# lewisjiang/contour-context

Hardware: AMD Instinct MI355X
Metric: scans/sec ingest+query (120k-pt scan vs 5k-scan DB); max-F1 parity (higher is better)
Workload: dtype f32+f64

## Files before the change

### contour-context_amd/csrc/cont2_amd.hip

```cpp
#include <hip/hip_runtime.h>

#include <algorithm>
#include <array>
#include <chrono>
#include <cstdlib>
#include <climits>
#include <cmath>
#include <cstdio>
#include <cstring>
#include <string>
#include <condition_variable>
#include <mutex>
#include <thread>
#include <vector>

#include "../../include/cont2_amd.h"
#include "cc_hostcfg.h"
#include "k_rasterize.h"
#include "k_contours.h"
#include "k_contours_list.h"
#include "k_knn.h"
#include "k_check.h"
#include "k_merge.h"
#include "k_gmm.h"
// ... 358 lines not shown
    double ph[9] = {0}, sub[8] = {0}, lv[6] = {0}, sa[4] = {0};
    for (int i = 0; i < n; i++) {
      const long long *p = &h[(size_t)i * CC_K2_NCLK];
      ph[0] += p[1] * 0.01;
      ph[1] += p[2] * 0.01;
      ph[2] += p[3] * 0.01;
      ph[3] += (p[5] - p[4]) * 0.01;
      ph[4] += (p[6] - p[5]) * 0.01;
      ph[5] += (p[7] - p[6]) * 0.01;
      ph[6] += (p[8] - p[7]) * 0.01;
      ph[7] += (p[8] - p[0]) * 0.01;
      sub[0] += (p[9] - p[0]) * 0.01;
      sub[1] += (p[11] - p[10]) * 0.01;
      sub[2] += (p[12] - p[11]) * 0.01;
      sub[3] += (p[4] - p[12]) * 0.01;
      sub[4] += p[14] * 0.01;
      sub[5] += p[15] * 0.01;
      for (int j = 0; j < 6; j++) lv[j] += p[16 + j] * 0.01;
      sa[0] += (p[22] - p[0]) * 0.01;
      sa[1] += (p[23] - p[22]) * 0.01;
      sa[2] += (p[24] - p[23]) * 0.01;
      sa[3] += (p[9] - p[24]) * 0.01;
    }
    fprintf(stderr, "[cc_k_contours phases, mean us over %d scans] ccl %.1f  enum+bbox %.1f  walk %.1f  order+sort %.1f  emit %.1f  keys %.1f  bci %.1f  | total %.1f\n",
            n, ph[0] / n, ph[1] / n, ph[2] / n, ph[3] / n, ph[4] / n, ph[5] / n, ph[6] / n, ph[7] / n);
    fprintf(stderr, "[cc_k_contours sub-phases] fill+list %.1f | walk: member lists %.1f  lane walk %.1f  eight-lane walk %.1f | keys: RoI lists %.1f  division sums %.1f\n",
            sub[0] / n, sub[1] / n, sub[2] / n, sub[3] / n, sub[4] / n, sub[5] / n);
    {
      cc_k2_big_queue hq;
      HIPCHK(hipMemcpy(&hq, c->main.d_midq, sizeof(hq), hipMemcpyDeviceToHost));
      fprintf(stderr, "[cc_k_contours] scans handed to the mid path so far: %d (configuration %d, cells / slots %d, components %d, list padding %d)\n", hq.total, hq.why[0], hq.why[1], hq.why[2], hq.why[3]);
    }
    fprintf(stderr, "[cc_k_contours list stage A] levels %.1f  chunk ballots %.1f  prefix %.1f  entries + run labels %.1f\n", sa[0] / n, sa[1] / n, sa[2] / n, sa[3] / n);
    fprintf(stderr, "[cc_k_contours level loop, summed over the levels] unions %.1f  flatten+count %.1f  kept roots %.1f  rank %.1f  bbox/area %.1f  records %.1f\n",
            lv[0] / n, lv[1] / n, lv[2] / n, lv[3] / n, lv[4] / n, lv[5] / n);
  }
  ms_out[0] = c->ms_acc[0];
  ms_out[1] = c->ms_acc[1];
  if (n_launches) *n_launches = c->launches;
  c->ms_acc[0] = c->ms_acc[1] = 0;
  c->launches = 0;
  return CC_OK;
}

int cc_destroy(cc_ctx *c) {
#ifdef CC_TUNE_K1_CLK
  {
    unsigned long long h[8] = {0};
    if (hipMemcpyFromSymbol(h, HIP_SYMBOL(cc_k1_clk), sizeof h) == hipSuccess)
      fprintf(stderr, "[cc_k_rasterize clocks, ticks of 10 ns summed over workgroups (thread 0)] init %llu | A %llu | barrier %llu | B %llu | barrier %llu | emit %llu\n", h[0], h[1], h[2],
              h[3], h[4], h[5]);
  }
#endif
  if (!c) return CC_OK;
  hipSetDevice(c->device);
  for (auto &e : c->ev) hipEventDestroy(e);
  for (auto &ch : c->chan) {
    if (ch.s) {
      stream_give(c->device, ch.s);
    }
    hipFree(ch.d_pts);
    hipFree(ch.d_desc_tmp);
    hipFree(ch.d_bev_copy);
    scratch_free(ch.scr);
  }
  scratch_free(c->main);
  for (int i = 0; i < cc_ctx::NSLOT; i++) {
// ... 573 lines not shown
```

### contour-context_amd/csrc/k_contours.h

```cpp
#pragma once
#include "cc_dev.h"
#include "cc_group.h"
#include "cc_sort.h"
#include "cc_stats.h"
#include "cc_fmath.h"

#ifndef CC_OPAQUE_I
#define CC_OPAQUE_I(x) asm volatile("" : "+v"(x))
#endif

#define CC_NC CC_MAXC
#define CC_LAB_NONE 0xFFFFu
#define CC_LAB_PENDING 0x7FFEu

struct cc_comp_t {
  uint16_t root, area, parent, rank;
  uint8_t r0, r1, c0, c1, cA, cB, pad[2];
};

template <int NC>
struct cc_k2_scratch_t {
  cc_comp_t comp[CC_NLEV][NC];
  cc_contour_t cont[CC_NLEV][NC];
  alignas(16) uint16_t memb[CC_NLEV][((CC_MAX_CELLS + 7) & ~7) + 8 * NC];
// ... 143 lines not shown
    if (phase_clk) {                                                                      \
      const long long now_ = (long long)wall_clock64();                                   \
      if (tid == 0) phase_clk[(size_t)scan * CC_K2_NCLK + 16 + (j)] += now_ - tsub; \
      tsub = now_;                                                                        \
    }                                                                                     \
  } while (0)
#define CC_K2_LAP(acc)                                     \
  do {                                                     \
    if (phase_clk) {                                       \
      const long long now_ = (long long)wall_clock64();    \
      acc += now_ - tmark;                                 \
      tmark = now_;                                        \
    }                                                      \
  } while (0)

struct cc_k2_levmap {
  const unsigned char *LV;
  const unsigned long long *bitmap;
  const uint16_t *cbase;
  const unsigned char *lev;
  const uint16_t *g_rc;
  const float2 *g_pix;
  int n_act;
};
template <bool LISTED>
__device__ __forceinline__ int cc_k2_lev_at(const cc_k2_levmap &M, int cell) {
  if (!LISTED) return (int)M.LV[cell];
  const unsigned long long m = M.bitmap[cell >> 6];
  const int bit = cell & 63;
  if (!((m >> bit) & 1ull)) return 0;
  return (int)M.lev[(int)M.cbase[cell >> 6] + __popcll(m & ((1ull << bit) - 1ull))];
}

template <int NC, bool BIG, bool LISTED>
__device__ __forceinline__ void cc_k2_back(const cc_dev_cfg &cfg, const float2 *__restrict__ pix, const cc_k1_scan_out *__restrict__ k1_out,
                                           cc_k2_scratch_t<NC> *__restrict__ scr, cc_k2_big_tables *__restrict__ bigtab, int scan,
                                           cc_scan_desc_t *__restrict__ desc_out, int16_t *__restrict__ labels_dbg, long long *__restrict__ phase_clk,
                                           char *R, const int *n_lev_in, int flags_in, const cc_k2_levmap &lm) {
  const int n_cell = cfg.n_cell, n_col = cfg.n_col, n_row = cfg.n_row;
  const int tid = threadIdx.x, nt = blockDim.x;
  const int wave_id = tid >> 6, lane = tid & 63, n_waves = nt >> 6;
  cc_scan_desc_t *desc = desc_out + scan;
  long long tmark = 0;
  int n_lev[CC_NLEV];
  for (int l = 0; l < CC_NLEV; l++) n_lev[l] = n_lev_in[l];
#define CC_NLEV_AT(i) ((i) == 0 ? n_lev[0] : (i) == 1 ? n_lev[1] : (i) == 2 ? n_lev[2] : (i) == 3 ? n_lev[3] : (i) == 4 ? n_lev[4] : n_lev[5])
  const int flags0 = flags_in;
  cc_comp_t *T = BIG ? bigtab->T : (cc_comp_t *)R;
  unsigned *skey = BIG ? bigtab->skey : (unsigned *)(R + 30720);
  unsigned *arr = BIG ? bigtab->arr : (unsigned *)(R + 30720 + 7680);
  cc_anchor_lds *top = (cc_anchor_lds *)(R + 30720 + 2 * 7680);
  int *sh2 = (int *)(R + 30720 + 2 * 7680 + 1280);
  char *R2 = R + 30720 + 2 * 7680 + 1280 + 256;
  for (int l = 0; l < CC_NLEV; l++)
    for (int k = tid; k < n_lev[l]; k += nt) T[l * NC + k] = scr->comp[l][k];
  __syncthreads();
  for (int l = 0; l < CC_NLEV; l++) {
    const int n = n_lev[l];
    for (int k = tid; k < n; k += nt) {
      const cc_comp_t cp = T[l * NC + k];
      int py0 = 0, px0 = 0, prank = 0;
      if (l > 0) {
        unsigned p = cp.parent;
        if (p < (unsigned)n_lev[l - 1]) {
          const cc_comp_t pp = T[(l - 1) * NC + p];
          py0 = pp.r0;
          px0 = pp.c0;
          prank = pp.rank;
        }
      }
      const int rmin = cp.r0;
      const int brow = (rmin - py0) >> 1;
      const int ra = py0 + 2 * brow;
      int cm = cp.cA;
      if (ra == rmin && cp.cB < cm) cm = cp.cB;
      const int bcol = (cm - px0) >> 1;
      skey[l * NC + k] = ((unsigned)prank << 14) | ((unsigned)brow << 7) | (unsigned)bcol;
    }
    __syncthreads();
    for (int k0 = 0; k0 < n; k0 += nt >> 2) {
      const int k = k0 + (tid >> 2), q = tid & 3;
      const unsigned me = k < n ? skey[l * NC + k] : 0u;
      int rk = 0;
      for (int j = q; j < n; j += 4) rk += (skey[l * NC + j] < me) ? 1 : 0;
      rk += __shfl_xor(rk, 1);
      rk += __shfl_xor(rk, 2);
// ... 13 lines not shown
        [&]() {
          for (int k = lane; k < n; k += 64) a[T[l * NC + k].rank] = ((unsigned)T[l * NC + k].area << 16) | (unsigned)k;
        },
        lane, lpos, rasc, skey + l * NC, (unsigned *)R2 + l * CC_SORT_STACK);
    int tot = 0;
    for (int i = lane; i < n; i += 64) tot += (int)(a[i] >> 16);
    for (int o = 32; o > 0; o >>= 1) tot += __shfl_xor(tot, o);
    if (lane == 0) sh2[l] = tot;
  }
  __syncthreads();
  CC_K2_STAMP(5);
  for (int l = 0; l < CC_NLEV; l++) {
    const int n = n_lev[l] < CC_MAXC ? n_lev[l] : CC_MAXC;
    const int n_words = n * (int)(sizeof(cc_contour_t) / 4);
    const unsigned *src = (const unsigned *)&scr->cont[l][0];
    unsigned *dst = (unsigned *)&desc->cont[l][0];
    for (int w = tid; w < n_words; w += nt) {
      const int seq = w / 19, off = w - seq * 19;
      const int k = (int)(arr[l * NC + seq] & 0xFFFFu);
      dst[w] = src[k * 19 + off];
    }
    for (int seq = tid; seq < CC_NDIST && seq < n; seq += nt) {
      const int k = (int)(arr[l * NC + seq] & 0xFFFFu);
      const cc_contour_t *cv = &scr->cont[l][k];
      cc_anchor_lds a;
      a.pm[0] = cv->pos_mean[0];
      a.pm[1] = cv->pos_mean[1];
      a.ev[0] = cv->eig_vals[0];
      a.ev[1] = cv->eig_vals[1];
      a.cnt = cv->cell_cnt;
      top[l * CC_NDIST + seq] = a;
    }
  }
  if (tid < CC_NLEV) {
    desc->n_cont[tid] = CC_NLEV_AT(tid);
    desc->n_stored[tid] = CC_NLEV_AT(tid) < CC_MAXC ? CC_NLEV_AT(tid) : CC_MAXC;
    desc->layer_cell_cnt[tid] = sh2[tid];
  }
  if (tid == 0) {
    const cc_k1_scan_out k1 = k1_out[scan];
    desc->max_bin_val = k1.max_bin_val;
    desc->min_bin_val = k1.min_bin_val;
    desc->n_pix = k1.n_pix;
    int fl = flags0;
    for (int l = 0; l < CC_NLEV; l++) fl |= n_lev[l] > CC_MAXC ? CC_DESC_TRUNCATED : 0;
    desc->flags = fl;
  }
  if (labels_dbg) {
    for (int l = 0; l < CC_NLEV; l++)
      for (int seq = tid; seq < n_lev[l]; seq += nt) skey[l * NC + (arr[l * NC + seq] & 0xFFFFu)] = (unsigned)seq;
    __syncthreads();
    for (int l = 0; l < CC_NLEV; l++) {
      int16_t *ld = labels_dbg + ((size_t)scan * CC_NLEV + l) * n_cell;
      for (int c = tid; c < n_cell; c += nt) {
        int16_t v = ld[c];
        if (v >= 0) ld[c] = (int16_t)skey[l * NC + v];
      }
    }
  }
  __syncthreads();

  CC_K2_STAMP(6);
  float *divs = (float *)R2;
  int *cntp = (int *)(R2 + 5056);
  int *valid = cntp + 36;
  int *accum = valid + 36;
  const int NA = CC_NLEV * CC_NPIV;
  if (tid < NA) {
    const int ll = tid / CC_NPIV, seq = tid - ll * CC_NPIV;
    int ok = 0, acc = 0;
    if (seq < cfg.piv_firsts) {
      for (int s = 0; s <= seq; s++)
        if (s < CC_NLEV_AT(ll)) acc += top[ll * CC_NDIST + s].cnt;
      ok = (seq < CC_NLEV_AT(ll) && top[ll * CC_NDIST + seq].cnt >= cfg.min_cont_key_cnt) ? 1 : 0;
    }
    valid[tid] = ok;
    accum[tid] = acc;
    cntp[tid] = 0;
  }
  double *exp_tab = (double *)(R2 + 5504);
  unsigned char *vlist = (unsigned char *)(R2 + 5504 + 512);
  if (tid >= 64 && tid < 128) exp_tab[tid - 64] = __longlong_as_double((long long)cc_exp2_tab64[tid - 64]);
  __syncthreads();
  int NV = 0;
  for (int a = 0; a < CC_NLEV * CC_NPIV; a++) {
    const int ok = valid[a];
    if (ok && tid == 0) vlist[NV] = (unsigned char)a;
    NV += ok;
  }
  __syncthreads();
  const int roi_pad = (int)ceilf(cfg.roi_radius + 1.f);
  const float div_len = cfg.roi_radius / (float)(7 * 5);
  const float bin_len = cfg.roi_radius / (float)7;
  const double r_lim = (double)cfg.roi_radius - 1e-2;
// ... 239 lines not shown
      if (lane == 0) {
        bcnt[a] = n;
        ob->dist_bin[0] = bw[0];
        ob->dist_bin[1] = bw[1];
        ob->dist_bin[2] = bw[2];
        ob->dist_bin[3] = bw[3];
        ob->piv_seq = seq < cfg.piv_firsts ? (int8_t)seq : (int8_t)0;
        ob->level = seq < cfg.piv_firsts ? (int8_t)ll : (int8_t)0;
        ob->n_pts = (uint8_t)n;
        ob->n_segs = (uint8_t)ns;
      }
    }
  }
  __syncthreads();
  for (int t = tid; t < NA * CC_BCI_MAXPTS; t += nt) {
    const int a = t / CC_BCI_MAXPTS, i = t - a * CC_BCI_MAXPTS;
    const int ll = a / CC_NPIV, seq = a - ll * CC_NPIV;
    unsigned w0 = 0u;
    float r = 0.f, th = 0.f;
    if (i < bcnt[a]) {
      const unsigned k = bkey[a * CC_BCI_MAXPTS + i];
      const int q = (int)(k & 0xFFu);
      const bci_tmp o = btmp[a * CC_BCI_MAXPTS + q];
      w0 = (unsigned)(q / CC_NDIST + 1) | ((unsigned)(q % CC_NDIST) << 8) | ((k >> 8) << 16);
      r = o.r;
      th = o.theta;
    }
    unsigned *dst = (unsigned *)&desc->bcis[ll][seq].pts[i];
    dst[0] = w0;
    dst[1] = __float_as_uint(r);
    dst[2] = __float_as_uint(th);
  }
  CC_K2_STAMP(8);
}

template <int NC, bool BIG>
__device__ __forceinline__ void cc_k2_body(const cc_dev_cfg &cfg, const float *__restrict__ bev_in, const float2 *__restrict__ pix_in,
                                           const cc_k1_scan_out *__restrict__ k1_out, cc_k2_scratch_t<NC> *__restrict__ scr,
                                           cc_k2_big_tables *__restrict__ bigtab, cc_k2_big_queue *__restrict__ queue, int scan,
                                           cc_scan_desc_t *__restrict__ desc_out, int16_t *__restrict__ labels_dbg, long long *__restrict__ phase_clk,
                                           char *smem) {
  CC_K2_STAMP(0);
  const int n_cell = cfg.n_cell, n_col = cfg.n_col, n_row = cfg.n_row;
  const int tid = threadIdx.x, nt = blockDim.x;

  unsigned char *LV = (unsigned char *)smem;
  char *R = smem + CC_K2_LV_BYTES(n_cell);
  uint16_t *LAB = (uint16_t *)R;
  unsigned *W = BIG ? bigtab->W : (unsigned *)(R + 45056);
  uint16_t *roots = BIG ? bigtab->roots : (uint16_t *)(R + 45056 + 8960);
  uint16_t *cand = BIG ? bigtab->cand : roots + NC;
  uint16_t *prev_root = BIG ? bigtab->prev_root : cand + NC;
  int *sh = (int *)(R + 45056 + 8960 + 3 * CC_NC * 2 + 64);

  const float *bev = bev_in + (size_t)scan * n_cell;
  const float2 *pix = pix_in + (size_t)scan * n_cell;
  cc_scan_desc_t *desc = desc_out + scan;

  {
    const float4 *bev4 = (const float4 *)bev;
    const int n_quad = n_cell >> 2;
#pragma unroll 6
    for (int v = tid; v < n_quad; v += nt) {
      const float4 h4 = bev4[v];
      const float hh[4] = {h4.x, h4.y, h4.z, h4.w};
      unsigned lv4 = 0;
// ... 658 lines not shown
```

### contour-context_amd/csrc/k_contours_list.h

```cpp
#pragma once
#include "k_contours.h"

#define CC_K2L_NCAP CC_LIST_CAP
#define CC_K2L_SCAP 12800
#ifndef CC_K2L_MEMB
#define CC_K2L_MEMB 11264
#endif
#define CC_K2L_BIG 64
#define CC_K2L_WL_CAP (CC_K2L_MEMB / 2)
#define CC_K2L_NSTR (CC_K2L_NCAP / 64)
#define CC_K2L_NCHUNK ((CC_MAX_CELLS + 63) / 64)
#define CC_K2L_O_BITMAP 0
#define CC_K2L_O_CBASE 2816
#define CC_K2L_O_LEV 3584
#define CC_K2L_O_REST 6656
#define CC_K2L_R_RC 0
#define CC_K2L_R_X 6144
#define CC_K2L_R_MEMB 43008
#define CC_K2L_R_AREA (CC_K2L_R_MEMB + 2 * CC_K2L_MEMB)
#define CC_K2L_R_PTR (CC_K2L_R_AREA + 3840)
#define CC_K2L_R_SH (CC_K2L_R_PTR + 3840)
#define CC_K2L_LDS_BYTES (CC_K2L_O_REST + CC_K2L_R_SH + 1024)
#define CC_K2L_X_OFF (2 * CC_K2L_SCAP)
#define CC_K2L_X_BITA (CC_K2L_X_OFF + 2 * CC_K2L_NCAP + 16)
#define CC_K2L_X_BITB (CC_K2L_X_BITA + CC_K2L_SCAP / 8)
static_assert(CC_K2L_SCAP / CC_K2L_BIG <= 256 && CC_K2L_BIG == 64 && CC_K2L_SCAP % 32 == 0 && CC_K2L_X_BITA % 4 == 0 && CC_K2L_SCAP < 0x8000 && CC_K2L_NSTR <= 64 && CC_NC * CC_NLEV * 2 == 3840, "list front half: table sizes");
static_assert(CC_K2L_X_BITB + CC_K2L_SCAP / 8 <= 36864 && CC_K2L_NCAP * 12 <= 36864, "list front half: region X / stage A overlays");
static_assert(CC_K2L_R_SH >= CC_K2_R_BYTES, "the back half's region");

#ifdef CC_EMU
#define CC_K2L_TRACE_BAIL() do { if (getenv("CC_EMU_TRACE_K2")) fprintf(stderr, "[k2 list] scan %d handed to the mid path (line %d)\n", scan, __LINE__); } while (0)
#else
#define CC_K2L_TRACE_BAIL() do { } while (0)
#endif

__device__ __forceinline__ int cc_k2l_idx_of(const unsigned long long *bitmap, const uint16_t *cbase, int cell) {
  const unsigned long long m = bitmap[cell >> 6];
  const int bit = cell & 63;
  return ((m >> bit) & 1ull) ? (int)cbase[cell >> 6] + __popcll(m & ((1ull << bit) - 1ull)) : -1;
}

__device__ __forceinline__ unsigned cc_uf_find_h(uint16_t *LAB, unsigned x) {
  for (;;) {
    const unsigned p = cc_lds_vread16(LAB + x);
    if (p == x) return x;
    const unsigned gp = cc_lds_vread16(LAB + p);
    if (gp == p) return p;
    cc_lds_vwrite16(LAB + x, gp);
    x = gp;
  }
}
__device__ __forceinline__ void cc_uf_union_h(uint16_t *LAB, unsigned a, unsigned b) {
  a = cc_uf_find_h(LAB, a);
  b = cc_uf_find_h(LAB, b);
  while (a != b) {
    if (a < b) {
      const unsigned t = a;
      a = b;
      b = t;
    }
    unsigned *w = (unsigned *)LAB + (a >> 1);
// ... 41 lines not shown

  unsigned long long *bitmap = (unsigned long long *)(smem + CC_K2L_O_BITMAP);
  uint16_t *cbase = (uint16_t *)(smem + CC_K2L_O_CBASE);
  unsigned char *lev = (unsigned char *)(smem + CC_K2L_O_LEV);
  char *R = smem + CC_K2L_O_REST;
  uint16_t *rc = (uint16_t *)(R + CC_K2L_R_RC);
  char *X = R + CC_K2L_R_X;
  uint16_t *LAB = (uint16_t *)X;
  uint16_t *off = (uint16_t *)(X + CC_K2L_X_OFF);
  unsigned *bitA = (unsigned *)(X + CC_K2L_X_BITA), *bitB = (unsigned *)(X + CC_K2L_X_BITB);
  uint16_t *memb = (uint16_t *)(R + CC_K2L_R_MEMB);
  unsigned *wl = (unsigned *)(R + CC_K2L_R_MEMB);
  uint16_t *area = (uint16_t *)(R + CC_K2L_R_AREA);
  uint16_t *ptr = (uint16_t *)(R + CC_K2L_R_PTR);
  int *sh = (int *)(R + CC_K2L_R_SH);
  unsigned char *scnt = (unsigned char *)(R + CC_K2L_R_SH + 512);
  uint16_t *big = (uint16_t *)(R + CC_K2L_R_SH + 512);

  const float *bev = bev_in + (size_t)scan * n_cell;
  const float2 *pix = pix_in + (size_t)scan * n_cell;
  long long acc_ccl = 0, acc_enum = 0, acc_walk = 0, tmark = phase_clk ? (long long)wall_clock64() : 0, tsub = tmark;
  if (phase_clk && tid == 0)
    for (int j = 0; j < 6; j++) phase_clk[(size_t)scan * CC_K2_NCLK + 16 + j] = 0;

  const int4 hd = list.hdr[scan];
  const int n_act = hd.x, n_slot = hd.y;
#ifdef CC_EMU
  if (tid == 0 && getenv("CC_EMU_TRACE_K2")) fprintf(stderr, "[k2 list] scan %d: %d active cells, %d slots\n", scan, n_act, n_slot);
#endif
  if (n_act > CC_K2L_NCAP || n_slot > CC_K2L_SCAP) CC_K2L_BAIL(1);
  const int n_chunk = (n_cell + 63) >> 6;
  const int n_str = (n_act + 63) >> 6;
  uint16_t *ssum = (uint16_t *)scnt;
  {
    const uint16_t *g_rc = list.rc + (size_t)scan * CC_LIST_CAP;
    const unsigned char *g_lev = list.lev + (size_t)scan * CC_LIST_CAP;
    for (int i = tid; i < n_act; i += nt) {
      rc[i] = g_rc[i];
      lev[i] = g_lev[i];
    }
    for (int i = tid; i < n_chunk; i += nt) bitmap[i] = 0ull;
    if (tid < 128) sh[tid] = 0;
    if (labels_dbg)
      for (int i = tid; i < CC_NLEV * n_cell; i += nt) labels_dbg[(size_t)scan * CC_NLEV * n_cell + i] = (int16_t)-1;
  }
  __syncthreads();
  CC_K2_STAMP(22);
  for (int i = tid; i < n_act; i += nt) {
    const unsigned rcv = rc[i];
    const int c = (int)(rcv >> 8) * n_col + (int)(rcv & 255u);
    atomicOr(&bitmap[c >> 6], 1ull << (c & 63));
  }
  for (int q = wave_id; q < n_str; q += n_waves) {
    const int i = q * 64 + lane;
    int v = i < n_act ? (int)lev[i] : 0;
    for (int o = 32; o > 0; o >>= 1) v += __shfl_xor(v, o);
    if (lane == 0) ssum[q] = (uint16_t)v;
  }
  __syncthreads();
  CC_K2_STAMP(23);
  {
    const unsigned long long lane_le = lane_lt | (1ull << lane);
    int spre;
    {
      const int v = lane < n_str ? (int)ssum[lane] : 0;
      const int incl = cc_wave_scan_incl(v);
// ... 143 lines not shown
        LAB[oi + l] = (uint16_t)rt;
        const unsigned bit = 1u << (rt & 31u);
        if (atomicOr(&bitA[rt >> 5], bit) & bit) atomicOr(&bitB[rt >> 5], bit);
      }
    }
  }
  __syncthreads();
  CC_K2_SUBLAP(1);
  CC_K2_LAP(acc_ccl);
#define CC_K2L_KEPT(s_) (need <= 1 || (((need == 2 ? bitA : bitB)[(s_) >> 5] >> ((s_) & 31)) & 1u))
  for (int q = wave_id; q < n_str; q += n_waves) {
    const int i = q * 64 + lane;
    const int Li = i < n_act ? (int)lev[i] : 0, oi = i < n_act ? (int)off[i] : 0;
#pragma unroll
    for (int l = 0; l < CC_NLEV; l++) {
      const bool kp = l < Li && (unsigned)LAB[oi + l] == (unsigned)(oi + l) && CC_K2L_KEPT(oi + l);
      const unsigned long long m = __ballot(kp);
      if (lane == 0) scnt[l * CC_K2L_NSTR + q] = (unsigned char)__popcll(m);
    }
  }
  __syncthreads();
  CC_K2_SUBLAP(2);
  int nk[CC_NLEV], pre[CC_NLEV];
  bool too_many = false;
#pragma unroll
  for (int l = 0; l < CC_NLEV; l++) {
    const int v = lane < n_str ? (int)scnt[l * CC_K2L_NSTR + lane] : 0;
    const int incl = cc_wave_scan_incl(v);
    pre[l] = incl - v;
    nk[l] = cc_wave_scan_total(incl);
    too_many = too_many || nk[l] > NC;
  }
  if (too_many) CC_K2L_BAIL(2);
  for (int q = wave_id; q < n_str; q += n_waves) {
    const int i = q * 64 + lane;
    const int Li = i < n_act ? (int)lev[i] : 0, oi = i < n_act ? (int)off[i] : 0;
#pragma unroll
    for (int l = 0; l < CC_NLEV; l++) {
      const bool kp = l < Li && (unsigned)LAB[oi + l] == (unsigned)(oi + l) && CC_K2L_KEPT(oi + l);
      const unsigned long long m = __ballot(kp);
      const int base = __builtin_amdgcn_readlane(pre[l], q);
      if (kp) LAB[oi + l] = (uint16_t)(0x8000u | (unsigned)(base + cc_mbcnt(m)));
    }
  }
  __syncthreads();
  CC_K2_SUBLAP(3);
  for (int i = tid; i < n_act; i += nt) {
    const int Li = (int)lev[i], oi = (int)off[i];
    int16_t *ld = nullptr;
    int cell = 0;
    if (labels_dbg) {
      const unsigned rcv = rc[i];
      cell = (int)(rcv >> 8) * n_col + (int)(rcv & 255u);
      ld = labels_dbg + (size_t)scan * CC_NLEV * n_cell;
    }
    unsigned jprev = 0xFFFFu;
    for (int l = 0; l < Li; l++) {
      const unsigned v = LAB[oi + l];
      unsigned j = CC_COMP_NONE;
      if (v & 0x8000u) {
        j = v & 0x7FFFu;
        if (l > 0) scr->comp[l][j].parent = (uint16_t)jprev;
      } else if (v != (unsigned)(oi + l)) {
        const unsigned rv = LAB[v];
        if (rv & 0x8000u) {
          j = rv & 0x7FFFu;
          LAB[oi + l] = (uint16_t)rv;
        }
      }
      if (j != CC_COMP_NONE) {
        const unsigned t = (unsigned)(l * NC) + j;
        atomicAdd((unsigned *)area + (t >> 1), 1u << ((t & 1u) * 16));
        if (ld) ld[(size_t)l * n_cell + cell] = (int16_t)j;
      }
      jprev = j == CC_COMP_NONE ? 0xFFFFu : j;
    }
  }
  __syncthreads();
  CC_K2_SUBLAP(4);
  CC_K2_LAP(acc_enum);
#define CC_K2L_NK(l_) ((l_) == 0 ? nk[0] : (l_) == 1 ? nk[1] : (l_) == 2 ? nk[2] : (l_) == 3 ? nk[3] : (l_) == 4 ? nk[4] : nk[5])
  CC_K2_STAMP(10);
  for (int l = wave_id; l < CC_NLEV; l += n_waves) {
    const int n = CC_K2L_NK(l);
    int run = 0;
    for (int k0 = 0; k0 < n; k0 += 64) {
      const int k = k0 + lane;
      const int a = k < n ? (int)area[l * NC + k] : 0;
      const int a4 = (a + 1) & ~1;
      const int incl = cc_wave_scan_incl(a4);
      if (k < n) {
        ptr[l * NC + k] = (uint16_t)(run + incl - a4);
        const int cls = a >= CC_K2L_BIG ? 7 : 31 - __clz(a);
        atomicAdd(&sh[32 + cls], 1);
      }
      run += cc_wave_scan_total(incl);
    }
    if (lane == 0) sh[16 + l] = run;
  }
  __syncthreads();
  int lbase[CC_NLEV + 1];
  lbase[0] = 0;
#pragma unroll
  for (int l = 0; l < CC_NLEV; l++) lbase[l + 1] = lbase[l] + sh[16 + l];
  if (lbase[CC_NLEV] > CC_K2L_MEMB) CC_K2L_BAIL(3);
#define CC_K2L_LBASE(l_) ((l_) == 0 ? lbase[0] : (l_) == 1 ? lbase[1] : (l_) == 2 ? lbase[2] : (l_) == 3 ? lbase[3] : (l_) == 4 ? lbase[4] : lbase[5])
  float ch[CC_K2L_NCAP / CC_K2_BLOCK];
  float2 cp[CC_K2L_NCAP / CC_K2_BLOCK];
  static_assert(CC_K2L_NCAP % CC_K2_BLOCK == 0, "entries per thread");
#pragma unroll
  for (int u = 0; u < CC_K2L_NCAP / CC_K2_BLOCK; u++) {
    const int i = tid + u * CC_K2_BLOCK;
    ch[u] = 0.f;
    cp[u] = make_float2(0.f, 0.f);
// ... 45 lines not shown
        M &= bit ? B : ~B;
      }
      const int rank = cc_mbcnt(M), total = __popcll(M);
      const bool last = (M >> lane) == 1ull;
      int base = 0;
      if (j != CC_COMP_NONE) {
        base = (int)ptr_l[j];
        ml[base + rank] = (uint16_t)i;
      }
      cc_wave_sync();
      if (j != CC_COMP_NONE && last) ptr_l[j] = (uint16_t)(base + total);
      cc_wave_sync();
    }
  }
  __threadfence_block();
  __syncthreads();
  float *cbev = (float *)X;
  float2 *cpix = (float2 *)(X + CC_K2L_NCAP * 4);
#pragma unroll
  for (int u = 0; u < CC_K2L_NCAP / CC_K2_BLOCK; u++) {
    const int i = tid + u * CC_K2_BLOCK;
    if (i < n_act) {
      cbev[i] = ch[u];
      cpix[i] = cp[u];
    }
  }
  __syncthreads();
  CC_K2_STAMP(11);
  int lev_base[CC_NLEV + 1];
  lev_base[0] = 0;
#pragma unroll
  for (int l = 0; l < CC_NLEV; l++) lev_base[l + 1] = lev_base[l] + nk[l];
  const int n_tot = lev_base[CC_NLEV];
  auto finish_stats = [&](int l, int k, int a, const uint16_t *ml, const cc_running_stat &rec) {
    const unsigned rcl = rc[ml[a - 1]];
    cc_contour_t cvw;
    cc_calc_stat_vals(cfg, rec, l, (int)(rcl >> 8), (int)(rcl & 255u), &cvw);
    scr->cont[l][k] = cvw;
  };
  auto finish_shape = [&](int l, int k, int a, const uint16_t *ml, int c0, int c1, int cB) {
    const unsigned rc0 = rc[ml[0]];
    cc_comp_t *cpo = &scr->comp[l][k];
    const unsigned root_cell = (rc0 >> 8) * (unsigned)n_col + (rc0 & 255u);
    *(unsigned *)cpo = root_cell | ((unsigned)a << 16);
    cpo->rank = 0;
    cpo->r0 = (uint8_t)(rc0 >> 8);
    cpo->r1 = 0;
    cpo->c0 = (uint8_t)c0;
    cpo->c1 = (uint8_t)c1;
    cpo->cA = (uint8_t)(rc0 & 255u);
    cpo->cB = (uint8_t)cB;
    cpo->pad[0] = cpo->pad[1] = 0;
  };
  const int n_big = sh[40 + 7];
  const int half = nt >> 1;
  const bool lane_walker = tid < half || nt < 128;
  const int wt = nt < 128 ? tid : (tid < half ? tid : tid - half), wn = nt < 128 ? nt : half;
  if (lane_walker)
  for (int g = wt; g < n_big; g += wn) {
    const int t_ = (int)big[g];
    const int l = t_ / NC, k = t_ - l * NC;
    const int a = (int)area[t_];
    const uint16_t *ml = memb + CC_K2L_LBASE(l) + (int)ptr[t_] - a;
    const unsigned *mlw = (const unsigned *)ml;
    const int row1 = (int)(rc[ml[0]] >> 8) + 1;
    int c0 = 255, c1 = 0, cB = 255;
    for (int m0 = 0; m0 < a; m0 += 8) {
      const unsigned wds[4] = {mlw[m0 >> 1], mlw[(m0 >> 1) + 1], mlw[(m0 >> 1) + 2], mlw[(m0 >> 1) + 3]};
      const int nv = a - m0;
      unsigned rcu[8];
#pragma unroll
      for (int u = 0; u < 8; u++) rcu[u] = rc[((wds[u >> 1] >> ((u & 1) * 16)) & 0xFFFFu) & (unsigned)-(int)(u < nv)];
#pragma unroll
      for (int u = 0; u < 8; u++) {
        const int col = (int)(rcu[u] & 255u);
        if (u < nv) {
          c0 = col < c0 ? col : c0;
          c1 = col > c1 ? col : c1;
          cB = ((int)(rcu[u] >> 8) == row1 && col < cB) ? col : cB;
        }
      }
    }
    finish_shape(l, k, a, ml, c0, c1, cB);
  }
  const int n_small = n_tot - n_big;
  if (lane_walker)
  for (int w = wt; w < n_small; w += wn) {
    const int t_ = (int)scr->act[w];
    const int l = t_ / NC, k = t_ - l * NC;
    const int a = (int)area[t_];
    const uint16_t *ml = memb + CC_K2L_LBASE(l) + (int)ptr[t_] - a;
    const unsigned *mlw = (const unsigned *)ml;
    cc_running_stat rec;
    rec.cnt = a;
    rec.ps_x = rec.ps_y = rec.t_xx = rec.t_xy = rec.t_yy = rec.tq_x = rec.tq_y = 0.0;
    rec.vol3 = 0.f;
    const int row1 = (int)(rc[ml[0]] >> 8) + 1;
    int c0 = 255, c1 = 0, cB = 255;
    unsigned nx[4] = {mlw[0], mlw[1], mlw[2], mlw[3]};
    for (int m0 = 0; m0 < a; m0 += 8) {
      const unsigned wds[4] = {nx[0], nx[1], nx[2], nx[3]};
      if (m0 + 8 < a) {
#pragma unroll
        for (int u = 0; u < 4; u++) nx[u] = mlw[(m0 >> 1) + 4 + u];
      }
      const int nv = a - m0;
      unsigned mk[8], rcu[8];
      float hv[8];
      float2 rv[8];
#pragma unroll
      for (int u = 0; u < 8; u++) {
        mk[u] = (unsigned)-(int)(u < nv);
        const unsigned iu = ((wds[u >> 1] >> ((u & 1) * 16)) & 0xFFFFu) & mk[u];
        hv[u] = cbev[iu];
        rv[u] = cpix[iu];
        rcu[u] = rc[iu];
      }
#pragma unroll
      for (int u = 0; u < 8; u++) {
        const float h = __uint_as_float(__float_as_uint(hv[u]) & mk[u]);
        const double vr = (double)__uint_as_float(__float_as_uint(rv[u].x) & mk[u]);
        const double vc = (double)__uint_as_float(__float_as_uint(rv[u].y) & mk[u]);
        rec.ps_x += vr;
        rec.ps_y += vc;
        rec.t_xx += vr * vr;
        rec.t_xy += vr * vc;
        rec.t_yy += vc * vc;
        rec.vol3 += h;
        rec.tq_x += (double)h * vr;
        rec.tq_y += (double)h * vc;
        const int col = (int)(rcu[u] & 255u);
        const int colm = mk[u] ? col : 255;
        c0 = colm < c0 ? colm : c0;
        c1 = (mk[u] && col > c1) ? col : c1;
        cB = (mk[u] && (int)(rcu[u] >> 8) == row1 && cB == 255) ? col : cB;
      }
    }
    finish_stats(l, k, a, ml, rec);
    finish_shape(l, k, a, ml, c0, c1, cB);
  }
  CC_K2_STAMP(12);
  {
    const int role = tid & 7;
    const unsigned fa_h = role >= 5 ? ~0u : 0u, fa_y = (role == 1 || role == 4) ? ~0u : 0u, fa_x = ~(fa_h | fa_y);
    const unsigned fb_1 = role < 2 ? ~0u : 0u, fb_x = (role == 2 || role == 5) ? ~0u : 0u, fb_y = ~(fb_1 | fb_x);
    if (!lane_walker || nt < 128)
    for (int g0 = 0; g0 < n_big; g0 += wn >> 3) {
      const int g = g0 + (wt >> 3);
      const bool on = g < n_big;
      double acc = 0.0;
      float vol3 = 0.f;
      int l = 0, k = 0, a = 0;
      const uint16_t *ml = memb;
      if (on) {
        const int t = (int)big[g];
        l = t / NC;
        k = t - l * NC;
        a = (int)area[t];
        ml = memb + CC_K2L_LBASE(l) + (int)ptr[t] - a;
        const unsigned *mlw = (const unsigned *)ml;
        unsigned nx[4] = {mlw[0], mlw[1], mlw[2], mlw[3]};
        for (int m0 = 0; m0 < a; m0 += 8) {
          const unsigned wds[4] = {nx[0], nx[1], nx[2], nx[3]};
          if (m0 + 8 < a) {
#pragma unroll
            for (int u = 0; u < 4; u++) nx[u] = mlw[(m0 >> 1) + 4 + u];
          }
          const int nv = a - m0;
          unsigned mk[8];
          float hv[8];
          float2 rv[8];
#pragma unroll
// ... 25 lines not shown
      rec.vol3 = vol3;
      rec.cnt = a;
      if (on && role == 0) finish_stats(l, k, a, ml, rec);
    }
  }
  CC_K2_LAP(acc_walk);
  if (phase_clk && tid == 0) {
    phase_clk[(size_t)scan * CC_K2_NCLK + 1] = acc_ccl;
    phase_clk[(size_t)scan * CC_K2_NCLK + 2] = acc_enum;
    phase_clk[(size_t)scan * CC_K2_NCLK + 3] = acc_walk;
  }
  CC_K2_STAMP(4);
#pragma unroll
  for (int l = 0; l < CC_NLEV; l++) n_lev_out[l] = nk[l];
  return true;
#undef CC_K2L_BAIL
#undef CC_K2L_KEPT
#undef CC_K2L_NK
#undef CC_K2L_LBASE
}

__global__ void __launch_bounds__(CC_K2_BLOCK, 4)
cc_k_contours(cc_dev_cfg cfg, const float *__restrict__ bev_in, const float2 *__restrict__ pix_in,
              const cc_k1_scan_out *__restrict__ k1_out, cc_k2_scratch *__restrict__ scratch_all,
              cc_scan_desc_t *__restrict__ desc_out, int16_t *__restrict__ labels_dbg, long long *__restrict__ phase_clk,
              cc_k2_big_queue *__restrict__ midq, cc_k1_list_out list) {
  HIP_DYNAMIC_SHARED(char, smem)
  const int scan = (int)blockIdx.x;
  cc_k2_scratch *scr = scratch_all + scan;
  int n_lev[CC_NLEV];
  if (!cc_k2_front_list(cfg, bev_in, pix_in, scr, midq, scan, desc_out, labels_dbg, phase_clk, smem, n_lev, list)) return;
  __threadfence_block();
  __syncthreads();
  cc_k2_levmap lm;
  lm.LV = nullptr;
  lm.bitmap = (const unsigned long long *)(smem + CC_K2L_O_BITMAP);
  lm.cbase = (const uint16_t *)(smem + CC_K2L_O_CBASE);
  lm.lev = (const unsigned char *)(smem + CC_K2L_O_LEV);
  lm.g_rc = list.rc + (size_t)scan * CC_LIST_CAP;
  lm.g_pix = list.pix + (size_t)scan * CC_LIST_CAP;
  lm.n_act = list.hdr[scan].x;
  cc_k2_back<CC_NC, false, true>(cfg, pix_in + (size_t)scan * cfg.n_cell, k1_out, scr, nullptr, scan, desc_out, labels_dbg, phase_clk,
                                 smem + CC_K2L_O_REST, n_lev, 0, lm);
}

__global__ void __launch_bounds__(CC_K2_BLOCK, 2)
cc_k_contours_mid(cc_dev_cfg cfg, float *bev_io, float2 *pix_io ,
                  const cc_k1_scan_out *__restrict__ k1_out, cc_k2_scratch *__restrict__ scratch_all, cc_k2_big_queue *__restrict__ midq,
                  cc_k2_big_queue *__restrict__ bigq, cc_scan_desc_t *__restrict__ desc_out, int16_t *__restrict__ labels_dbg,
                  int *__restrict__ seen ,
                  cc_k1_list_out list) {
  HIP_DYNAMIC_SHARED(char, smem)
  __shared__ int s_next;
  if (midq->n_flagged == 0) {
    if (blockIdx.x == 0 && threadIdx.x == 0) *seen = 0;
    return;
  }
  for (;;) {
    __syncthreads();
    if (threadIdx.x == 0) s_next = atomicAdd(&midq->next, 1);
    __syncthreads();
    const int k = s_next;
    if (k >= midq->n_flagged) {
      if (threadIdx.x == 0 && atomicAdd(&midq->exited, 1) == (int)gridDim.x - 1) {
        *seen = midq->n_flagged;
        midq->n_flagged = 0;
        midq->next = 0;
        midq->exited = 0;
      }
      return;
    }
    const int scan = midq->scan[k];
    const int4 hd = list.hdr[scan];
    if (hd.z == 0) {
#ifdef CC_EMU
      if (threadIdx.x == 0 && getenv("CC_EMU_TRACE_K2")) fprintf(stderr, "[k2 mid] scan %d: dense image rebuilt from the list (%d entries)\n", scan, hd.x);
// ... 49 lines not shown
```

Baseline: 598,800.

## Order and sort contours inside the list kernel, write records directly to descriptor

The list contour kernel now computes each kept component's geometry (top row, min column, row-below min column) with atomics during the label pass. It then ranks components by parent-relative position and sorts them by area in shared memory. Contour statistics are written straight into the output descriptor at their final sequence index, so the separate back-half pass (copy to scratch, rank, sort, gather) is skipped. This also removes the per-component member walks for shape bounds and the extra global scratch traffic. In exchange it adds LDS atomics and an O(n^2/4) rank loop, and it relies on new shared-memory overlays that must not collide.

```diff
diff --git a/contour-context_amd/csrc/cont2_amd.hip b/contour-context_amd/csrc/cont2_amd.hip
--- a/contour-context_amd/csrc/cont2_amd.hip
+++ b/contour-context_amd/csrc/cont2_amd.hip
@@ -414,7 +414,7 @@
       fprintf(stderr, "[cc_k_contours] scans handed to the mid path so far: %d (configuration %d, cells / slots %d, components %d, list padding %d)\n", hq.total, hq.why[0], hq.why[1], hq.why[2], hq.why[3]);
     }
     fprintf(stderr, "[cc_k_contours list stage A] levels %.1f  chunk ballots %.1f  prefix %.1f  entries + run labels %.1f\n", sa[0] / n, sa[1] / n, sa[2] / n, sa[3] / n);
-    fprintf(stderr, "[cc_k_contours level loop, summed over the levels] unions %.1f  flatten+count %.1f  kept roots %.1f  rank %.1f  bbox/area %.1f  records %.1f\n",
+    fprintf(stderr, "[cc_k_contours level loop, summed over the levels] unions %.1f  flatten+count %.1f  kept roots %.1f  rank %.1f  bbox/area %.1f  records (list kernel: order + sort) %.1f\n",
             lv[0] / n, lv[1] / n, lv[2] / n, lv[3] / n, lv[4] / n, lv[5] / n);
   }
   ms_out[0] = c->ms_acc[0];
diff --git a/contour-context_amd/csrc/k_contours.h b/contour-context_amd/csrc/k_contours.h
--- a/contour-context_amd/csrc/k_contours.h
+++ b/contour-context_amd/csrc/k_contours.h
@@ -199,6 +199,33 @@
   return (int)M.lev[(int)M.cbase[cell >> 6] + __popcll(m & ((1ull << bit) - 1ull))];
 }
 
+#define CC_K2_R_TOP (30720 + 2 * 7680)
+
+__device__ __forceinline__ void cc_k2_header(const cc_k1_scan_out *__restrict__ k1_out, int scan, cc_scan_desc_t *__restrict__ desc,
+                                             const int *n_lev, const int *lcc, int flags0) {
+  const int tid = threadIdx.x;
+#define CC_NLEV_AT(i) ((i) == 0 ? n_lev[0] : (i) == 1 ? n_lev[1] : (i) == 2 ? n_lev[2] : (i) == 3 ? n_lev[3] : (i) == 4 ? n_lev[4] : n_lev[5])
+  if (tid < CC_NLEV) {
+    desc->n_cont[tid] = CC_NLEV_AT(tid);
+    desc->n_stored[tid] = CC_NLEV_AT(tid) < CC_MAXC ? CC_NLEV_AT(tid) : CC_MAXC;
+    desc->layer_cell_cnt[tid] = lcc[tid];
+  }
+#undef CC_NLEV_AT
+  if (tid == 0) {
+    const cc_k1_scan_out k1 = k1_out[scan];
+    desc->max_bin_val = k1.max_bin_val;
+    desc->min_bin_val = k1.min_bin_val;
+    desc->n_pix = k1.n_pix;
+    int fl = flags0;
+    for (int l = 0; l < CC_NLEV; l++) fl |= n_lev[l] > CC_MAXC ? CC_DESC_TRUNCATED : 0;
+    desc->flags = fl;
+  }
+}
+
+template <bool LISTED>
+__device__ __forceinline__ void cc_k2_keys_bci(const cc_dev_cfg &cfg, const float2 *__restrict__ pix, int scan, cc_scan_desc_t *__restrict__ desc,
+                                               long long *__restrict__ phase_clk, char *R, const int *n_lev_in, const cc_k2_levmap &lm);
+
 template <int NC, bool BIG, bool LISTED>
 __device__ __forceinline__ void cc_k2_back(const cc_dev_cfg &cfg, const float2 *__restrict__ pix, const cc_k1_scan_out *__restrict__ k1_out,
                                            cc_k2_scratch_t<NC> *__restrict__ scr, cc_k2_big_tables *__restrict__ bigtab, int scan,
@@ -216,9 +243,9 @@
   cc_comp_t *T = BIG ? bigtab->T : (cc_comp_t *)R;
   unsigned *skey = BIG ? bigtab->skey : (unsigned *)(R + 30720);
   unsigned *arr = BIG ? bigtab->arr : (unsigned *)(R + 30720 + 7680);
-  cc_anchor_lds *top = (cc_anchor_lds *)(R + 30720 + 2 * 7680);
-  int *sh2 = (int *)(R + 30720 + 2 * 7680 + 1280);
-  char *R2 = R + 30720 + 2 * 7680 + 1280 + 256;
+  cc_anchor_lds *top = (cc_anchor_lds *)(R + CC_K2_R_TOP);
+  int *sh2 = (int *)(R + CC_K2_R_TOP + 1280);
+  char *R2 = R + CC_K2_R_TOP + 1280 + 256;
   for (int l = 0; l < CC_NLEV; l++)
     for (int k = tid; k < n_lev[l]; k += nt) T[l * NC + k] = scr->comp[l][k];
   __syncthreads();
@@ -298,20 +325,7 @@
       top[l * CC_NDIST + seq] = a;
     }
   }
-  if (tid < CC_NLEV) {
-    desc->n_cont[tid] = CC_NLEV_AT(tid);
-    desc->n_stored[tid] = CC_NLEV_AT(tid) < CC_MAXC ? CC_NLEV_AT(tid) : CC_MAXC;
-    desc->layer_cell_cnt[tid] = sh2[tid];
-  }
-  if (tid == 0) {
-    const cc_k1_scan_out k1 = k1_out[scan];
-    desc->max_bin_val = k1.max_bin_val;
-    desc->min_bin_val = k1.min_bin_val;
-    desc->n_pix = k1.n_pix;
-    int fl = flags0;
-    for (int l = 0; l < CC_NLEV; l++) fl |= n_lev[l] > CC_MAXC ? CC_DESC_TRUNCATED : 0;
-    desc->flags = fl;
-  }
+  cc_k2_header(k1_out, scan, desc, n_lev, sh2, flags0);
   if (labels_dbg) {
     for (int l = 0; l < CC_NLEV; l++)
       for (int seq = tid; seq < n_lev[l]; seq += nt) skey[l * NC + (arr[l * NC + seq] & 0xFFFFu)] = (unsigned)seq;
@@ -325,7 +339,23 @@
     }
   }
   __syncthreads();
-
+  cc_k2_keys_bci<LISTED>(cfg, pix, scan, desc, phase_clk, R, n_lev, lm);
+#undef CC_NLEV_AT
+}
+
+template <bool LISTED>
+__device__ __forceinline__ void cc_k2_keys_bci(const cc_dev_cfg &cfg, const float2 *__restrict__ pix, int scan, cc_scan_desc_t *__restrict__ desc,
+                                               long long *__restrict__ phase_clk, char *R, const int *n_lev_in, const cc_k2_levmap &lm) {
+  const int n_cell = cfg.n_cell, n_col = cfg.n_col, n_row = cfg.n_row;
+  const int tid = threadIdx.x, nt = blockDim.x;
+  const int wave_id = tid >> 6, lane = tid & 63, n_waves = nt >> 6;
+  long long tmark = 0;
+  int n_lev[CC_NLEV];
+  for (int l = 0; l < CC_NLEV; l++) n_lev[l] = n_lev_in[l];
+#define CC_NLEV_AT(i) ((i) == 0 ? n_lev[0] : (i) == 1 ? n_lev[1] : (i) == 2 ? n_lev[2] : (i) == 3 ? n_lev[3] : (i) == 4 ? n_lev[4] : n_lev[5])
+  const cc_anchor_lds *top = (const cc_anchor_lds *)(R + CC_K2_R_TOP);
+  char *R2 = R + CC_K2_R_TOP + 1280 + 256;
+  (void)n_cell;
   CC_K2_STAMP(6);
   float *divs = (float *)R2;
   int *cntp = (int *)(R2 + 5056);
@@ -631,6 +661,7 @@
     dst[2] = __float_as_uint(th);
   }
   CC_K2_STAMP(8);
+#undef CC_NLEV_AT
 }
 
 template <int NC, bool BIG>
diff --git a/contour-context_amd/csrc/k_contours_list.h b/contour-context_amd/csrc/k_contours_list.h
--- a/contour-context_amd/csrc/k_contours_list.h
+++ b/contour-context_amd/csrc/k_contours_list.h
@@ -24,9 +24,17 @@
 #define CC_K2L_X_OFF (2 * CC_K2L_SCAP)
 #define CC_K2L_X_BITA (CC_K2L_X_OFF + 2 * CC_K2L_NCAP + 16)
 #define CC_K2L_X_BITB (CC_K2L_X_BITA + CC_K2L_SCAP / 8)
+#define CC_K2L_X_GEO (CC_K2L_X_BITA + 4 * CC_NLEV * CC_NC)
+#define CC_K2L_X_C0 (CC_K2L_X_GEO + 2 * CC_NLEV * CC_NC)
+#define CC_K2L_X_CB (CC_K2L_X_C0 + 4 * CC_NLEV * CC_NC)
+#define CC_K2L_X_STK (CC_K2L_X_CB + 4 * CC_NLEV * CC_NC)
 static_assert(CC_K2L_SCAP / CC_K2L_BIG <= 256 && CC_K2L_BIG == 64 && CC_K2L_SCAP % 32 == 0 && CC_K2L_X_BITA % 4 == 0 && CC_K2L_SCAP < 0x8000 && CC_K2L_NSTR <= 64 && CC_NC * CC_NLEV * 2 == 3840, "list front half: table sizes");
 static_assert(CC_K2L_X_BITB + CC_K2L_SCAP / 8 <= 36864 && CC_K2L_NCAP * 12 <= 36864, "list front half: region X / stage A overlays");
 static_assert(CC_K2L_R_SH >= CC_K2_R_BYTES, "the back half's region");
+static_assert(CC_K2L_X_GEO >= CC_K2L_X_BITB + CC_K2L_SCAP / 8 && CC_K2L_X_GEO >= CC_K2L_R_MEMB - CC_K2L_R_X && CC_K2L_X_C0 % 4 == 0 &&
+              CC_K2L_X_STK + 4 * CC_NLEV * CC_SORT_STACK <= CC_K2L_R_AREA - CC_K2L_R_X && CC_NC <= 512 && 2 * CC_NC * 2 <= 4 * CC_NC,
+              "list front half: the ordering tables (GEO / C0 / CB are written in (D), while bitA / bitB are still read; they end "
+              "before the areas; a sort's two u16 lists fit a CB row)");
 
 #ifdef CC_EMU
 #define CC_K2L_TRACE_BAIL() do { if (getenv("CC_EMU_TRACE_K2")) fprintf(stderr, "[k2 list] scan %d handed to the mid path (line %d)\n", scan, __LINE__); } while (0)
@@ -134,6 +142,12 @@
   const int n_chunk = (n_cell + 63) >> 6;
   const int n_str = (n_act + 63) >> 6;
   uint16_t *ssum = (uint16_t *)scnt;
+  unsigned *ARR = (unsigned *)(X + CC_K2L_X_BITA);
+  uint16_t *GEO = (uint16_t *)(X + CC_K2L_X_GEO);
+  unsigned *C0 = (unsigned *)(X + CC_K2L_X_C0);
+  unsigned *CB = (unsigned *)(X + CC_K2L_X_CB);
+  unsigned *STK = (unsigned *)(X + CC_K2L_X_STK);
+  uint16_t *PAR = ptr;
   {
     const uint16_t *g_rc = list.rc + (size_t)scan * CC_LIST_CAP;
     const unsigned char *g_lev = list.lev + (size_t)scan * CC_LIST_CAP;
@@ -343,6 +357,7 @@
     too_many = too_many || nk[l] > NC;
   }
   if (too_many) CC_K2L_BAIL(2);
+#define CC_K2L_NK(l_) ((l_) == 0 ? nk[0] : (l_) == 1 ? nk[1] : (l_) == 2 ? nk[2] : (l_) == 3 ? nk[3] : (l_) == 4 ? nk[4] : nk[5])
   for (int q = wave_id; q < n_str; q += n_waves) {
     const int i = q * 64 + lane;
     const int Li = i < n_act ? (int)lev[i] : 0, oi = i < n_act ? (int)off[i] : 0;
@@ -351,27 +366,29 @@
       const bool kp = l < Li && (unsigned)LAB[oi + l] == (unsigned)(oi + l) && CC_K2L_KEPT(oi + l);
       const unsigned long long m = __ballot(kp);
       const int base = __builtin_amdgcn_readlane(pre[l], q);
-      if (kp) LAB[oi + l] = (uint16_t)(0x8000u | (unsigned)(base + cc_mbcnt(m)));
+      if (kp) {
+        const int j = base + cc_mbcnt(m);
+        LAB[oi + l] = (uint16_t)(0x8000u | (unsigned)j);
+        GEO[l * NC + j] = rc[i];
+        C0[l * NC + j] = 255u;
+        CB[l * NC + j] = 255u;
+      }
     }
   }
   __syncthreads();
   CC_K2_SUBLAP(3);
   for (int i = tid; i < n_act; i += nt) {
     const int Li = (int)lev[i], oi = (int)off[i];
-    int16_t *ld = nullptr;
-    int cell = 0;
-    if (labels_dbg) {
-      const unsigned rcv = rc[i];
-      cell = (int)(rcv >> 8) * n_col + (int)(rcv & 255u);
-      ld = labels_dbg + (size_t)scan * CC_NLEV * n_cell;
-    }
+    const unsigned rcv = rc[i];
+    const int col = (int)(rcv & 255u), row = (int)(rcv >> 8);
+    const int lw = (col > 0 && i > 0 && (unsigned)rc[i - 1] == rcv - 1u) ? (int)lev[i - 1] : 0;
     unsigned jprev = 0xFFFFu;
     for (int l = 0; l < Li; l++) {
       const unsigned v = LAB[oi + l];
       unsigned j = CC_COMP_NONE;
       if (v & 0x8000u) {
         j = v & 0x7FFFu;
-        if (l > 0) scr->comp[l][j].parent = (uint16_t)jprev;
+        if (l > 0) PAR[l * NC + j] = (uint16_t)jprev;
       } else if (v != (unsigned)(oi + l)) {
         const unsigned rv = LAB[v];
         if (rv & 0x8000u) {
@@ -382,15 +399,100 @@
       if (j != CC_COMP_NONE) {
         const unsigned t = (unsigned)(l * NC) + j;
         atomicAdd((unsigned *)area + (t >> 1), 1u << ((t & 1u) * 16));
-        if (ld) ld[(size_t)l * n_cell + cell] = (int16_t)j;
+        if (l >= lw) {
+          atomicMin(&C0[t], (unsigned)col);
+          if (row == (int)(GEO[t] >> 8) + 1) atomicMin(&CB[t], (unsigned)col);
+        }
       }
       jprev = j == CC_COMP_NONE ? 0xFFFFu : j;
     }
   }
   __syncthreads();
   CC_K2_SUBLAP(4);
+  for (int l = 0; l < CC_NLEV; l++) {
+    const int n = CC_K2L_NK(l);
+    const int np = l > 0 ? CC_K2L_NK(l - 1) : 0;
+    for (int k = tid; k < n; k += nt) {
+      const int t = l * NC + k;
+      int py0 = 0, px0 = 0, prank = 0;
+      if (l > 0) {
+        const unsigned p = PAR[t];
+        if (p < (unsigned)np) {
+          const unsigned pc = C0[(l - 1) * NC + p];
+          py0 = (int)(GEO[(l - 1) * NC + p] >> 8);
+          px0 = (int)(pc & 255u);
+          prank = (int)(pc >> 16);
+        }
+      }
+      const unsigned g = GEO[t];
+      const int rmin = (int)(g >> 8);
+      const int brow = (rmin - py0) >> 1;
+      const int ra = py0 + 2 * brow;
+      int cm = (int)(g & 255u);
+      const int cb = (int)CB[t];
+      if (ra == rmin && cb < cm) cm = cb;
+      const int bcol = (cm - px0) >> 1;
+      CB[t] = ((unsigned)prank << 14) | ((unsigned)brow << 7) | (unsigned)bcol;
+    }
+    __syncthreads();
+    for (int k0 = 0; k0 < n; k0 += nt >> 2) {
+      const int k = k0 + (tid >> 2), q = tid & 3;
+      const unsigned me = k < n ? CB[l * NC + k] : 0u;
+      int rk = 0;
+      for (int j = q; j < n; j += 4) rk += (CB[l * NC + j] < me) ? 1 : 0;
+      rk += __shfl_xor(rk, 1);
+      rk += __shfl_xor(rk, 2);
+      if (k < n && q == 0) {
+        C0[l * NC + k] |= (unsigned)rk << 16;
+        ARR[l * NC + rk] = ((unsigned)area[l * NC + k] << 16) | (unsigned)k;
+      }
+    }
+    __syncthreads();
+  }
+  for (int l = wave_id; l < CC_NLEV; l += n_waves) {
+    unsigned *a = ARR + l * NC;
+    const int n = CC_K2L_NK(l);
+    unsigned short *lpos = (unsigned short *)(CB + l * NC), *rasc = lpos + NC;
+    ccsort::std_sort_wave(
+        a, n, [](unsigned x) { return 0xFFFFu - (x >> 16); },
+        [&]() {
+          for (int k = lane; k < n; k += 64) a[C0[l * NC + k] >> 16] = ((unsigned)area[l * NC + k] << 16) | (unsigned)k;
+        },
+        lane, lpos, rasc, CB + l * NC, STK + l * CC_SORT_STACK);
+    int tot = 0;
+    for (int i = lane; i < n; i += 64) tot += (int)(a[i] >> 16);
+    for (int o = 32; o > 0; o >>= 1) tot += __shfl_xor(tot, o);
+    if (lane == 0) sh[48 + l] = tot;
+  }
+  __syncthreads();
+  for (int t = tid; t < CC_NLEV * NC; t += nt) {
+    const int l = t / NC, seq = t - l * NC;
+    if (seq < CC_K2L_NK(l)) {
+      const unsigned v = ARR[t];
+      GEO[l * NC + (int)(v & 0xFFFFu)] = (uint16_t)seq;
+      area[t] = (uint16_t)(v >> 16);
+    }
+  }
+  __syncthreads();
+  for (int i = tid; i < n_act; i += nt) {
+    const int Li = (int)lev[i], oi = (int)off[i];
+    int16_t *ld = nullptr;
+    if (labels_dbg) {
+      const unsigned rcv = rc[i];
+      ld = labels_dbg + (size_t)scan * CC_NLEV * n_cell + (int)(rcv >> 8) * n_col + (int)(rcv & 255u);
+    }
+    for (int l = 0; l < Li; l++) {
+      const unsigned v = LAB[oi + l];
+      if (v & 0x8000u) {
+        const unsigned seq = GEO[l * NC + (int)(v & 0x7FFFu)];
+        LAB[oi + l] = (uint16_t)(0x8000u | seq);
+        if (ld) ld[(size_t)l * n_cell] = (int16_t)seq;
+      }
+    }
+  }
+  __syncthreads();
+  CC_K2_SUBLAP(5);
   CC_K2_LAP(acc_enum);
-#define CC_K2L_NK(l_) ((l_) == 0 ? nk[0] : (l_) == 1 ? nk[1] : (l_) == 2 ? nk[2] : (l_) == 3 ? nk[3] : (l_) == 4 ? nk[4] : nk[5])
   CC_K2_STAMP(10);
   for (int l = wave_id; l < CC_NLEV; l += n_waves) {
     const int n = CC_K2L_NK(l);
@@ -502,57 +604,17 @@
 #pragma unroll
   for (int l = 0; l < CC_NLEV; l++) lev_base[l + 1] = lev_base[l] + nk[l];
   const int n_tot = lev_base[CC_NLEV];
-  auto finish_stats = [&](int l, int k, int a, const uint16_t *ml, const cc_running_stat &rec) {
+  cc_contour_t *cont_out = &desc_out[scan].cont[0][0];
+  auto finish_stats = [&](int l, int seq, int a, const uint16_t *ml, const cc_running_stat &rec) {
     const unsigned rcl = rc[ml[a - 1]];
     cc_contour_t cvw;
     cc_calc_stat_vals(cfg, rec, l, (int)(rcl >> 8), (int)(rcl & 255u), &cvw);
-    scr->cont[l][k] = cvw;
-  };
-  auto finish_shape = [&](int l, int k, int a, const uint16_t *ml, int c0, int c1, int cB) {
-    const unsigned rc0 = rc[ml[0]];
-    cc_comp_t *cpo = &scr->comp[l][k];
-    const unsigned root_cell = (rc0 >> 8) * (unsigned)n_col + (rc0 & 255u);
-    *(unsigned *)cpo = root_cell | ((unsigned)a << 16);
-    cpo->rank = 0;
-    cpo->r0 = (uint8_t)(rc0 >> 8);
-    cpo->r1 = 0;
-    cpo->c0 = (uint8_t)c0;
-    cpo->c1 = (uint8_t)c1;
-    cpo->cA = (uint8_t)(rc0 & 255u);
-    cpo->cB = (uint8_t)cB;
-    cpo->pad[0] = cpo->pad[1] = 0;
+    if (seq < CC_MAXC) cont_out[l * CC_MAXC + seq] = cvw;
   };
   const int n_big = sh[40 + 7];
   const int half = nt >> 1;
   const bool lane_walker = tid < half || nt < 128;
   const int wt = nt < 128 ? tid : (tid < half ? tid : tid - half), wn = nt < 128 ? nt : half;
-  if (lane_walker)
-  for (int g = wt; g < n_big; g += wn) {
-    const int t_ = (int)big[g];
-    const int l = t_ / NC, k = t_ - l * NC;
-    const int a = (int)area[t_];
-    const uint16_t *ml = memb + CC_K2L_LBASE(l) + (int)ptr[t_] - a;
-    const unsigned *mlw = (const unsigned *)ml;
-    const int row1 = (int)(rc[ml[0]] >> 8) + 1;
-    int c0 = 255, c1 = 0, cB = 255;
-    for (int m0 = 0; m0 < a; m0 += 8) {
-      const unsigned wds[4] = {mlw[m0 >> 1], mlw[(m0 >> 1) + 1], mlw[(m0 >> 1) + 2], mlw[(m0 >> 1) + 3]};
-      const int nv = a - m0;
-      unsigned rcu[8];
-#pragma unroll
-      for (int u = 0; u < 8; u++) rcu[u] = rc[((wds[u >> 1] >> ((u & 1) * 16)) & 0xFFFFu) & (unsigned)-(int)(u < nv)];
-#pragma unroll
-      for (int u = 0; u < 8; u++) {
-        const int col = (int)(rcu[u] & 255u);
-        if (u < nv) {
-          c0 = col < c0 ? col : c0;
-          c1 = col > c1 ? col : c1;
-          cB = ((int)(rcu[u] >> 8) == row1 && col < cB) ? col : cB;
-        }
-      }
-    }
-    finish_shape(l, k, a, ml, c0, c1, cB);
-  }
   const int n_small = n_tot - n_big;
   if (lane_walker)
   for (int w = wt; w < n_small; w += wn) {
@@ -565,8 +627,6 @@
     rec.cnt = a;
     rec.ps_x = rec.ps_y = rec.t_xx = rec.t_xy = rec.t_yy = rec.tq_x = rec.tq_y = 0.0;
     rec.vol3 = 0.f;
-    const int row1 = (int)(rc[ml[0]] >> 8) + 1;
-    int c0 = 255, c1 = 0, cB = 255;
     unsigned nx[4] = {mlw[0], mlw[1], mlw[2], mlw[3]};
     for (int m0 = 0; m0 < a; m0 += 8) {
       const unsigned wds[4] = {nx[0], nx[1], nx[2], nx[3]};
@@ -575,7 +635,7 @@
         for (int u = 0; u < 4; u++) nx[u] = mlw[(m0 >> 1) + 4 + u];
       }
       const int nv = a - m0;
-      unsigned mk[8], rcu[8];
+      unsigned mk[8];
       float hv[8];
       float2 rv[8];
 #pragma unroll
@@ -584,7 +644,6 @@
         const unsigned iu = ((wds[u >> 1] >> ((u & 1) * 16)) & 0xFFFFu) & mk[u];
         hv[u] = cbev[iu];
         rv[u] = cpix[iu];
-        rcu[u] = rc[iu];
       }
 #pragma unroll
       for (int u = 0; u < 8; u++) {
@@ -599,15 +658,9 @@
         rec.vol3 += h;
         rec.tq_x += (double)h * vr;
         rec.tq_y += (double)h * vc;
-        const int col = (int)(rcu[u] & 255u);
-        const int colm = mk[u] ? col : 255;
-        c0 = colm < c0 ? colm : c0;
-        c1 = (mk[u] && col > c1) ? col : c1;
-        cB = (mk[u] && (int)(rcu[u] >> 8) == row1 && cB == 255) ? col : cB;
       }
     }
     finish_stats(l, k, a, ml, rec);
-    finish_shape(l, k, a, ml, c0, c1, cB);
   }
   CC_K2_STAMP(12);
   {
@@ -699,6 +752,29 @@
   if (!cc_k2_front_list(cfg, bev_in, pix_in, scr, midq, scan, desc_out, labels_dbg, phase_clk, smem, n_lev, list)) return;
   __threadfence_block();
   __syncthreads();
+  CC_K2_STAMP(5);
+  char *R = smem + CC_K2L_O_REST;
+  cc_scan_desc_t *desc = desc_out + scan;
+  cc_k2_header(k1_out, scan, desc, n_lev, (const int *)(R + CC_K2L_R_SH) + 48, 0);
+  {
+    cc_anchor_lds *top = (cc_anchor_lds *)(R + CC_K2_R_TOP);
+    const int t = threadIdx.x;
+    if (t < CC_NLEV * CC_NDIST) {
+      const int l = t / CC_NDIST, seq = t - l * CC_NDIST;
+      const int n = l == 0 ? n_lev[0] : l == 1 ? n_lev[1] : l == 2 ? n_lev[2] : l == 3 ? n_lev[3] : l == 4 ? n_lev[4] : n_lev[5];
+      if (seq < n) {
+        const cc_contour_t *cv = &desc->cont[l][seq];
+        cc_anchor_lds a;
+        a.pm[0] = cv->pos_mean[0];
+        a.pm[1] = cv->pos_mean[1];
+        a.ev[0] = cv->eig_vals[0];
+        a.ev[1] = cv->eig_vals[1];
+        a.cnt = cv->cell_cnt;
+        top[t] = a;
+      }
+    }
+  }
+  __syncthreads();
   cc_k2_levmap lm;
   lm.LV = nullptr;
   lm.bitmap = (const unsigned long long *)(smem + CC_K2L_O_BITMAP);
@@ -707,8 +783,7 @@
   lm.g_rc = list.rc + (size_t)scan * CC_LIST_CAP;
   lm.g_pix = list.pix + (size_t)scan * CC_LIST_CAP;
   lm.n_act = list.hdr[scan].x;
-  cc_k2_back<CC_NC, false, true>(cfg, pix_in + (size_t)scan * cfg.n_cell, k1_out, scr, nullptr, scan, desc_out, labels_dbg, phase_clk,
-                                 smem + CC_K2L_O_REST, n_lev, 0, lm);
+  cc_k2_keys_bci<true>(cfg, pix_in + (size_t)scan * cfg.n_cell, scan, desc, phase_clk, R, n_lev, lm);
 }
 
 __global__ void __launch_bounds__(CC_K2_BLOCK, 2)
```

After: 604,300, median of 6. Within noise of the previous version (+0.9%).
